# lincbrain/Fibers.jl

Hardware: AMD Instinct MI355X
Metric: Mvoxels/s fit (GQI ODF + peaks, 140^3 x 270-dir); Mpoints/s streamline in extra (higher is better)
Workload: dtype f32 (operands as 2 fp16 pieces = 23 bits on MFMA, 3 piece products, f32 accumulate); 1 GPU; gqi_rec + find_peaks + qa normalisation (gqi.jl:109-201), ONE 140x140x140 x 270-frame volume (18 x b=5 + 84 dirs x {1000,2000,3000}), sphere_642, all-ones mask; voxels=2744000, voxels_per_gpu=2744000, frames=270, odf_vertices=321, parallelism=single GPU

## Files before the change

### fibers.jl_amd/csrc/odf.hip

```cpp
#include <algorithm>
#include <cmath>
#include <type_traits>
#include <utility>

#include "common.h"

namespace {

typedef float f32x16 __attribute__((ext_vector_type(16)));

constexpr int KT = 16;
constexpr int WG_VOX = 128;

#include "odf_gemm_f32.inc"
#include "odf_fused_epilogue.inc"
#include "odf_gemm3.inc"
#include "odf_mask.inc"
#include "odf_peaks.inc"
#include "odf_post.inc"

}

struct fib_odf_plan {
    int device = 0;
    int nvol = 0, nvert = 0, nrows = 0, nrow0 = 0;
    int MB = 11, NX = 0, ntile_m = 1, Kpad = 0, maxdeg = 0;
    int scale_frame = -1;
    float scale_coef = 0.0f;
    bool has_ineff = false;
    int gM = 0, gK = 0, gRow0 = 0;
    std::vector<float> G;
    bool folded = false;
    int fold_span_max = 0, scale_frame_raw = -1;
    fib::DevBuf<int32_t> foldA, foldB;
    mutable fib::DevBuf<float> folded_dwi;
    std::vector<float> A;
    fib::DevBuf<float> At, verts;
    fib::DevBuf<uint16_t> At3;
    fib::DevBuf<float> Aextra;
    fib::DevBuf<float> Gdev;
    mutable fib::DevBuf<int32_t> inf_list;
    bool split_bf16 = false;
    bool h2 = false;
    float h2_sa = 1.0f;
    bool fused_shape = false;
    bool fused = false;
    bool dsi2_shape = false, dsi2 = false;
    int MBB = 0;
    fib::DevBuf<uint16_t> At3b;
    mutable fib::DevBuf<unsigned> pair_flags;
    fib::DevBuf<uint16_t> At3f;
    fib::DevBuf<float> Aextraf;
    mutable fib::DevBuf<float> mean_hi;
    mutable fib::DevBuf<int32_t> redo_list;
    fib::DevBuf<uint32_t> effbits;
    fib::DevBuf<int32_t> nbr, nbr64;
    int deg_pad = 6, rows_pad = 0;
    bool is_s642 = false;
    mutable fib::DevBuf<unsigned> maxenc;
    mutable fib::DevBuf<int32_t> live_vox, live_tiles, live_counts;
    mutable fib::DevBuf<unsigned long long> compact_state;
    mutable fib::DevBuf<unsigned long long> compact_sub;
    mutable fib::DevBuf<unsigned long long> compact_state2;
    mutable fib::DevBuf<unsigned> compact_mode;
    mutable fib::DevBuf<unsigned long long> compact_oct;
    mutable unsigned compact_epoch = 0;
    fib::DevBuf<unsigned> tickets;
    fib::DevBuf<unsigned> selctr;
    fib::DevBuf<unsigned long long> sellist;
    mutable fib::DevBuf<float> odfmax;
};

namespace {


int resolve_format(int format) {
    if (format != FIB_ODF_FORMAT_DEFAULT) return format;
    const char *e = fib::env("FIBERS_ODF_FORMAT");
    if (!e) {
        const char *g = fib::env("FIBERS_ODF_GEMM"), *x = fib::env("FIBERS_ODF_EXACT");
        if (g && (!strcmp(g, "f32") || !strcmp(g, "F32"))) return FIB_ODF_FORMAT_F32;
        if (x && x[0] != '\0' && x[0] != '0') return FIB_ODF_FORMAT_BF16X3;
    }
    if (e && (!strcmp(e, "f32") || !strcmp(e, "F32"))) return FIB_ODF_FORMAT_F32;
    if (e && (!strcmp(e, "bf16x3") || !strcmp(e, "BF16X3"))) return FIB_ODF_FORMAT_BF16X3;
    return FIB_ODF_FORMAT_FP16X2;
}

int finish_plan(fib_odf_plan *p, const float *verts, int nverts, const int32_t *faces, int nfaces,
                const std::vector<float> &frame_eff, int format = FIB_ODF_FORMAT_DEFAULT) {
    if (p->G.empty()) { p->G = p->A; p->gM = p->nrows; p->gK = p->nvol; p->gRow0 = p->nrow0; }
    const int M = p->gM, K = p->gK;
    format = resolve_format(format);
    p->split_bf16 = format != FIB_ODF_FORMAT_F32;
    int best_cost = INT32_MAX;
    const int nxs[] = {0, 1};
    for (int mb = p->split_bf16 ? 10 : 11; mb >= 5; mb--)
        for (int nx : nxs) {
            if (nx > 0 && mb > 10) continue;
            const int rows = mb * 32 + nx;
            const int nt = (M + rows - 1) / rows;
            const int cost = nt * (64 * mb + 4 * nx);
            if (cost < best_cost) { best_cost = cost; p->MB = mb; p->NX = nx; p->ntile_m = nt; }
        }
    p->Kpad = (K + KT - 1) / KT * KT;
    const int MW = gemm_row_stride(p->MB, p->NX), ROWS = p->MB * 32 + p->NX;
    std::vector<float> At((size_t)p->ntile_m * p->Kpad * MW, 0.0f);
    for (int k = 0; k < K; k++)
        for (int r = 0; r < M; r++) {
            const int tm = r / ROWS, rr = r % ROWS;
            At[((size_t)tm * p->Kpad + k) * MW + rr] = p->G[r + (size_t)M * k];
        }
    bool any_ineff = false;
    for (int k = 0; k < K; k++) if (frame_eff[k] == 0.0f) any_ineff = true;
    if (p->split_bf16 && (any_ineff || p->Kpad / KT < 2 || p->MB > 10 || (size_t)p->ntile_m * p->NX * p->Kpad > 2048)) p->split_bf16 = false;
    if (p->split_bf16) {
        p->h2 = format == FIB_ODF_FORMAT_FP16X2;
        float gmax = 0.0f;
// ... 254 lines not shown
            const float *cj = &p->A[(size_t)p->nrows * j], *ck = &p->A[(size_t)p->nrows * partner[j]];
            for (int r = 0; r < p->nrows && ok; r++) if (cj[r] != ck[r]) ok = false;
        }
        if (ok) {
            std::vector<int32_t> fa, fb;
            for (int j = 0; j < nvol; j++) if (j <= partner[j]) { fa.push_back(j); fb.push_back(partner[j] == j ? -1 : partner[j]); }
            const int nrep = (int)fa.size();
            p->folded = true; p->gK = nrep; p->gRow0 = nrep; p->gM = nrep + p->nvert;
            p->G.assign((size_t)p->gM * nrep, 0.0f);
            for (int c = 0; c < nrep; c++) {
                const float *col = &p->A[(size_t)p->nrows * fa[c]];
                for (int r = 0; r < nrep; r++) p->G[r + (size_t)p->gM * c] = col[fa[r]];
                for (int v = 0; v < p->nvert; v++) p->G[nrep + v + (size_t)p->gM * c] = col[nvol + v];
                if (fa[c] == p->scale_frame) p->scale_frame = -1000 - c;
            }
            if (p->scale_frame <= -1000) { p->scale_frame = -(p->scale_frame + 1000); p->scale_frame_raw = fa[p->scale_frame]; }
            for (int t0 = 0; t0 < nrep; t0 += KT)
                for (const std::vector<int32_t> *side : {&fa, &fb}) {
                    int lo = 1 << 30, hi = -1;
                    for (int j = t0; j < std::min(nrep, t0 + KT); j++) if ((*side)[j] >= 0) { lo = std::min(lo, (*side)[j]); hi = std::max(hi, (*side)[j]); }
                    if (hi >= 0) p->fold_span_max = std::max(p->fold_span_max, hi - lo + 1);
                }
            if ((rc = p->foldA.alloc(nrep)) != FIB_OK || (rc = p->foldB.alloc(nrep)) != FIB_OK) { delete p; return rc; }
            (void)hipMemcpy(p->foldA.p, fa.data(), nrep * sizeof(int32_t), hipMemcpyHostToDevice);
            (void)hipMemcpy(p->foldB.p, fb.data(), nrep * sizeof(int32_t), hipMemcpyHostToDevice);
            eff.assign((size_t)nrep, 1.0f);
        }
    }
    rc = finish_plan(p, verts, nverts, faces, nfaces, eff, format);
    if (rc != FIB_OK) { delete p; return rc; }
    *plan = p;
    return FIB_OK;
} FIB_API_CATCH

extern "C" void fib_odf_plan_destroy(fib_odf_plan *plan) try {
    if (!plan) return;
    fib::DeviceGuard guard;
    (void)hipSetDevice(plan->device);
    delete plan;
} FIB_API_CATCH_VOID

extern "C" int fib_odf_plan_matrix(const fib_odf_plan *plan, float *A, int *nrows, int *nvol, int *nvert) try {
    FIB_CHECK(plan != nullptr, FIB_ERR_INVALID, "plan is NULL");
    if (nrows) *nrows = plan->nrows;
    if (nvol) *nvol = plan->nvol;
    if (nvert) *nvert = plan->nvert;
    if (A) memcpy(A, plan->A.data(), plan->A.size() * sizeof(float));
    return FIB_OK;
} FIB_API_CATCH

namespace {

constexpr int FOLD_MB_MAX = 10;
template <int MB, int NX>
void launch_gemm(const GemmArgs &ga, unsigned grid, hipStream_t st) {
    if (ga.At3) {
        int ncu = 256, dev = 0;
        (void)hipGetDevice(&dev);
        (void)hipDeviceGetAttribute(&ncu, hipDeviceAttributeMultiprocessorCount, dev);
        GemmArgs g2 = ga;
        const int nw = 8;
        const int64_t items = fib::cdiv(ga.nvox, nw * 32) * ga.ntile_m;
        unsigned pg = (unsigned)std::min<int64_t>((int64_t)ncu * (8 / nw), items);
        pg = (pg + 7) / 8 * 8;
        auto go = [&](auto h2_) {
            constexpr bool H2 = decltype(h2_)::value;
            if (ga.fold) {
                if constexpr (MB <= FOLD_MB_MAX) hipLaunchKernelGGL((odf_gemm3_kernel<MB, NX, 8, true, false, H2>), dim3(pg), dim3(512), 0, st, g2);
                return;
            }
            if constexpr (MB == 10 && NX == 1) {
                if (ga.mean_hi) { hipLaunchKernelGGL((odf_gemm3_kernel<10, 1, 8, false, true, H2>), dim3(pg), dim3(512), 0, st, g2); return; }
            }
            hipLaunchKernelGGL((odf_gemm3_kernel<MB, NX, 8, false, false, H2>), dim3(pg), dim3(512), 0, st, g2);
        };
        if (ga.h2) go(std::true_type{}); else go(std::false_type{});
    }
    else hipLaunchKernelGGL((odf_gemm_kernel<MB, NX>), dim3(grid), dim3(256), 0, st, ga);
}

size_t peaks_smem(const fib_odf_plan *p) {
    return ((size_t)(p->rows_pad + 1) * PV + (size_t)PG * PV * PREC) * sizeof(float);
}

template <int DEG, bool EXACT>
int launch_peaks_t(const PeakArgs &pa, size_t smem, unsigned grid, hipStream_t st) {
    FIB_HIP(hipFuncSetAttribute(reinterpret_cast<const void *>(odf_peaks_kernel<DEG, EXACT>),
                                hipFuncAttributeMaxDynamicSharedMemorySize, (int)smem));
    hipLaunchKernelGGL((odf_peaks_kernel<DEG, EXACT>), dim3(grid), dim3(PW * 64), smem, st, pa);
    FIB_HIP(hipGetLastError());
    return FIB_OK;
}

template <int DEG, bool EXACT>
int launch_peaks64_t(const PeakArgs &pa, size_t smem, int64_t ntiles, unsigned grid, hipStream_t st) {
    FIB_HIP(hipFuncSetAttribute(reinterpret_cast<const void *>(odf_peaks64_kernel<DEG, EXACT>),
                                hipFuncAttributeMaxDynamicSharedMemorySize, (int)smem));
    hipLaunchKernelGGL((odf_peaks64_kernel<DEG, EXACT>), dim3(grid), dim3(P64_T), smem, st, pa, ntiles);
    FIB_HIP(hipGetLastError());
    return FIB_OK;
}

int launch_peaks(const fib_odf_plan *plan, const float *odf, int64_t nvox, int64_t stride, float *const peak[3], float *const qa[3],
                 int32_t *isort_top, int32_t *nvalid, bool reduce, hipStream_t st, bool small_tiles = false,
                 const int32_t *tiles = nullptr, const int32_t *ntl = nullptr) {
    PeakArgs pa{};
    pa.tiles = tiles; pa.ntl = ntl;
    pa.odf = odf; pa.nbr = plan->nbr.p; pa.nbr64 = plan->nbr64.p; pa.verts = plan->verts.p;
    for (int k = 0; k < 3; k++) { pa.peak[k] = peak ? peak[k] : nullptr; pa.qa[k] = qa ? qa[k] : nullptr; }
    pa.isort_top = isort_top; pa.nvalid = nvalid;
    pa.maxenc = reduce ? plan->maxenc.p : nullptr;
    pa.mean_hi = reduce ? plan->mean_hi.p : nullptr;
    pa.nvox = nvox; pa.stride = stride; pa.nvert = plan->nvert; pa.rows_pad = plan->rows_pad;
    pa.vec_ok = (stride % 4 == 0 && ((uintptr_t)odf & 15) == 0) ? 1 : 0;
    const size_t smem = peaks_smem(plan);
    FIB_CHECK(smem <= 160 * 1024, FIB_ERR_UNSUPPORTED, "ODF with %d vertices does not fit the peak finder's LDS tile", plan->nvert);
    const unsigned grid = (unsigned)fib::cdiv(nvox, PV);
    const bool exact = isort_top != nullptr;
    fib::ProfScope prof("odf_peaks", st);
    const size_t smem64 = ((size_t)(plan->nvert + 1) * 64 + (size_t)P64_W * 64 * PREC + (size_t)plan->nvert * (plan->deg_pad + 3)) * sizeof(float);
    if (!small_tiles && plan->nvert * 16 <= P64_NI * P64_T && smem64 <= 160 * 1024) {
        int ncu = 256;
        (void)hipDeviceGetAttribute(&ncu, hipDeviceAttributeMultiprocessorCount, plan->device);
        const int64_t ntiles = fib::cdiv(nvox, 64);
        const unsigned g64 = (unsigned)std::min<int64_t>(ntiles, ncu);
        if (plan->is_s642 && !exact) {
            const size_t smem642 = ((size_t)(FIB_S642_NVERT + 1) * 64 + (size_t)PQ_CAP * 64 * 2 + 128 + 2 * P64_W * 64 + 2 * 8 * 64 +
                                    (size_t)FIB_S642_NVERT * 3) * sizeof(float);
            FIB_HIP(hipFuncSetAttribute(reinterpret_cast<const void *>(odf_peaks642_kernel), hipFuncAttributeMaxDynamicSharedMemorySize, (int)smem642));
            hipLaunchKernelGGL(odf_peaks642_kernel, dim3(g64), dim3(P64_T), smem642, st, pa, ntiles);
            FIB_HIP(hipGetLastError());
            return FIB_OK;
        }
        switch (plan->deg_pad) {
            case 6:  return exact ? launch_peaks64_t<6, true>(pa, smem64, ntiles, g64, st) : launch_peaks64_t<6, false>(pa, smem64, ntiles, g64, st);
            case 8:  return exact ? launch_peaks64_t<8, true>(pa, smem64, ntiles, g64, st) : launch_peaks64_t<8, false>(pa, smem64, ntiles, g64, st);
            default: return exact ? launch_peaks64_t<16, true>(pa, smem64, ntiles, g64, st) : launch_peaks64_t<16, false>(pa, smem64, ntiles, g64, st);
        }
    }
    switch (plan->deg_pad) {
        case 6:  return exact ? launch_peaks_t<6, true>(pa, smem, grid, st) : launch_peaks_t<6, false>(pa, smem, grid, st);
        case 8:  return exact ? launch_peaks_t<8, true>(pa, smem, grid, st) : launch_peaks_t<8, false>(pa, smem, grid, st);
        default: return exact ? launch_peaks_t<16, true>(pa, smem, grid, st) : launch_peaks_t<16, false>(pa, smem, grid, st);
    }
}

}

namespace {
int launch_mask_compact(const fib_odf_plan *plan, const uint8_t *mask, int64_t nvox, unsigned *maxenc, const ZeroArgs *z, hipStream_t st) {
    int iters = (int)std::max<int64_t>(1, fib::cdiv(fib::cdiv(nvox, CB), 256));
    if (iters > CB_ITERS_MAX) iters = CB_ITERS_MAX;
    const int nchunks = (int)fib::cdiv(nvox, (int64_t)CB * iters);
    FIB_CHECK(nchunks <= 1024, FIB_ERR_UNSUPPORTED, "volume too large for the mask compaction");
    int rc;
    if ((rc = plan->live_vox.ensure((size_t)nvox)) != FIB_OK) return rc;
    if ((rc = plan->live_tiles.ensure((size_t)fib::cdiv(nvox, 64))) != FIB_OK) return rc;
    if (!plan->compact_state.p) {
        if ((rc = plan->compact_state.alloc(1024)) != FIB_OK) return rc;
        FIB_HIP(hipMemsetAsync(plan->compact_state.p, 0, 1024 * sizeof(unsigned long long), st));
    }
    if (!plan->compact_state2.p) {
        if ((rc = plan->compact_state2.alloc(1024)) != FIB_OK) return rc;
        FIB_HIP(hipMemsetAsync(plan->compact_state2.p, 0, 1024 * sizeof(unsigned long long), st));
        if ((rc = plan->compact_mode.alloc(2)) != FIB_OK) return rc;
        FIB_HIP(hipMemsetD32Async(reinterpret_cast<hipDeviceptr_t>(plan->compact_mode.p), 1, 2, st));
    }
    const size_t nsub = (size_t)fib::cdiv(nvox, CB);
    if (z && plan->compact_sub.n < nsub) {
        if ((rc = plan->compact_sub.alloc(nsub)) != FIB_OK) return rc;
        FIB_HIP(hipMemsetAsync(plan->compact_sub.p, 0, nsub * sizeof(unsigned long long), st));
    }
    if (++plan->compact_epoch == 0u) plan->compact_epoch = 1u;
    CompactArgs c{};
    c.mask = mask; c.nvox = nvox; c.vidx = plan->live_vox.p; c.tiles = plan->live_tiles.p; c.state = plan->compact_state.p;
    c.ticket = plan->tickets.p; c.totals = plan->live_counts.p; c.maxenc = maxenc; c.epoch = plan->compact_epoch; c.nchunks = nchunks; c.iters = iters;
    c.zero = z != nullptr;
    if (z) c.z = *z;
    c.clear = plan->pair_flags.p; c.nclear = plan->pair_flags.p ? 8 * 32 : 0;
    c.sub_state = plan->compact_sub.p;
    c.state2 = plan->compact_state2.p; c.mode = plan->compact_mode.p;
    const size_t noct = (size_t)fib::cdiv(nvox, 1024);
    if (z && noct * sizeof(unsigned) <= 48 * 1024) {
        if (plan->compact_oct.n < noct) {
            if ((rc = plan->compact_oct.alloc(noct)) != FIB_OK) return rc;
            FIB_HIP(hipMemsetAsync(plan->compact_oct.p, 0, noct * sizeof(unsigned long long), st));
        }
        c.oct_bits = plan->compact_oct.p; c.oct_words = (int)noct;
    }
    { const char *e = fib::ab_env("FIBERS_COMPACT_UNKNOWN"); c.dbg_unknown = e ? atoi(e) : 0; }
    { const char *e = fib::ab_env("FIBERS_ODF_LIST"); c.force = !e ? -1 : (e[0] == 'q' ? 0 : (e[0] == 'o' ? 1 : -1)); }
    fib::ProfScope prof("mask_compact", st);
    const int grid = nchunks + (z ? 256 : 0);
    hipLaunchKernelGGL(mask_compact_kernel, dim3(grid), dim3(1024), c.oct_words * sizeof(unsigned), st, c);
    FIB_HIP(hipGetLastError());
    return FIB_OK;
}
}

extern "C" int fibd_odf_rec(const fib_odf_plan *plan, const float *dwi, const uint8_t *mask, int64_t nvox,
                            float *pdf, float *odf, float *const peak[3], float *const qa[3],
                            float *odfmax_dev, int flags, void *stream) try {
    FIB_CHECK(plan && dwi && mask && odf && peak && qa, FIB_ERR_INVALID, "NULL argument");
    FIB_CHECK(nvox > 0, FIB_ERR_INVALID, "nvox must be positive");
    FIB_CHECK(nvox <= ((int64_t)1 << 27), FIB_ERR_UNSUPPORTED, "volumes of more than 2^27 voxels are not supported (32-bit lane offsets)");
    FIB_CHECK(plan->nrow0 == 0 || pdf != nullptr, FIB_ERR_INVALID, "DSI plans need a pdf output volume");
    for (int k = 0; k < 3; k++) FIB_CHECK(peak[k] && qa[k], FIB_ERR_INVALID, "NULL peak/qa output volume");
    fib::DeviceGuard guard;
    FIB_HIP(hipSetDevice(plan->device));
    hipStream_t st = (hipStream_t)stream;
    GemmArgs ga{};
    {
        ZeroArgs z{};
        z.out0 = pdf; z.out1 = odf; z.n0 = plan->nrow0; z.n1 = plan->nrows - plan->nrow0; z.nvox = nvox; z.stride = nvox;
        for (int k = 0; k < 3; k++) { z.peak[k] = peak[k]; z.qa[k] = qa[k]; }
        int rcc = launch_mask_compact(plan, mask, nvox, plan->maxenc.p, !(flags & FIB_ODF_PREZEROED) ? &z : nullptr, st);
        if (rcc != FIB_OK) return rcc;
    }
    ga.At = plan->At.p; ga.At3 = (plan->split_bf16 && nvox <= ((int64_t)1 << 26)) ? plan->At3.p : nullptr; ga.S = dwi;
    ga.Aextra = plan->Aextra.p; ga.h2 = plan->h2 ? 1 : 0; ga.h2_inv_sa = 1.0f / plan->h2_sa;
#ifdef FIB_CLOCK_STAMP
    { const char *pi = fib::ab_env("FIBERS_PHASE_ITEM"); ga.phase_item = pi ? atoi(pi) : 2; }
    { const char *pw = fib::ab_env("FIBERS_PHASE_WG"); ga.phase_wg = pw ? atoi(pw) : 8; }
#endif
    ga.vec_ok = (nvox % 4 == 0 && ((uintptr_t)odf & 15) == 0 && (pdf == nullptr || ((uintptr_t)pdf & 15) == 0)) ? 1 : 0; ga.vidx = plan->live_vox.p; ga.nlive = plan->live_counts.p; ga.mask = mask; ga.effbits = plan->effbits.p;
    ga.out0 = pdf; ga.out1 = odf; ga.nvox = nvox;
    if (ga.At3 && plan->Gdev.p) {
        int rci = plan->inf_list.ensure((size_t)nvox);
        if (rci != FIB_OK) return rci;
        ga.fix_count = plan->live_counts.p + 2; ga.fix_list = plan->inf_list.p; ga.fix_cap = (int)std::min<int64_t>(nvox, INT32_MAX);
    }
    const bool sep = (flags & FIB_ODF_SEPARATE_PEAKS) != 0;
    const bool fuse = plan->fused && ga.At3 != nullptr && ga.vec_ok && !sep;
    {
        int rcm = plan->mean_hi.ensure((size_t)nvox + 4);
        if (rcm != FIB_OK) return rcm;
    }
    auto setup_fused = [&]() -> int {
        int rcf = plan->redo_list.ensure((size_t)nvox);
        if (rcf != FIB_OK) return rcf;
        ga.At3 = plan->At3f.p; ga.Aextra = plan->Aextraf.p;
        for (int k = 0; k < 3; k++) { ga.peak[k] = peak[k]; ga.qa[k] = qa[k]; }
        ga.verts = plan->verts.p; ga.maxenc = plan->maxenc.p; ga.mean_hi = plan->mean_hi.p;
        ga.redo_count = plan->live_counts.p + 3; ga.redo_list = plan->redo_list.p; ga.redo_cap = (int)std::min<int64_t>(nvox, INT32_MAX);
        { const char *pa = fib::ab_env("FIBERS_ODF_ANTI"); ga.anti = pa ? atoi(pa) : 3; }
        return FIB_OK;
    };
    if (fuse) { int rcf = setup_fused(); if (rcf != FIB_OK) return rcf; }
    ga.K = plan->gK; ga.Kpad = plan->Kpad; ga.M = plan->gM; ga.nrow0 = plan->gRow0; ga.ntile_m = plan->ntile_m;
    const bool fold_ok = plan->folded && ga.At3 != nullptr && plan->Kpad <= FKMAX && plan->scale_frame_raw >= 0 &&
                         (int64_t)plan->fold_span_max * nvox * 4 < (int64_t)0xE0000000ll;
    const bool fuse_fold = fold_ok && plan->MB <= FOLD_MB_MAX;
    const bool dsi2 = plan->dsi2 && fold_ok && ga.vec_ok && !sep;
    if (dsi2) {
        int rcf = setup_fused();
        if (rcf != FIB_OK) return rcf;
        ga.At3b = plan->At3b.p;
        ga.ntile_m = 2;
    }
    if (fuse_fold || dsi2) {
        ga.fold = 1;
        ga.rowA = plan->foldA.p; ga.rowB = plan->foldB.p;
    } else if (plan->folded) {
        int rcf = plan->folded_dwi.ensure((size_t)plan->gK * nvox);
        if (rcf != FIB_OK) return rcf;
        fib::ProfScope prof("dsi_fold", st);
        if (nvox % 4 == 0 && ((uintptr_t)dwi & 15) == 0 && ((uintptr_t)mask & 3) == 0)
            hipLaunchKernelGGL(dsi_fold4_kernel, dim3((unsigned)fib::cdiv(nvox / 4, 256)), dim3(256), 0, st, dwi, mask, plan->foldA.p, plan->foldB.p,
                               plan->gK, nvox, plan->folded_dwi.p);
        else
            hipLaunchKernelGGL(dsi_fold_kernel, dim3((unsigned)fib::cdiv(nvox, 256)), dim3(256), 0, st, dwi, mask, plan->foldA.p, plan->foldB.p,
                               plan->gK, nvox, plan->folded_dwi.p);
        ga.S = plan->folded_dwi.p;
        ga.rowA = plan->foldA.p; ga.rowB = plan->foldB.p;
    }
    ga.scale_frame = plan->nrow0 > 0 ? ((fuse_fold || dsi2) ? plan->scale_frame_raw : plan->scale_frame) : -1;
    ga.scale_coef = plan->scale_coef;
    ga.stride = nvox;
    ga.has_ineff = plan->has_ineff ? 1 : 0;
    FIB_CHECK(fib::cdiv(nvox, WG_VOX) * plan->ntile_m < ((int64_t)1 << 31), FIB_ERR_UNSUPPORTED, "volume too large for one launch");

    auto run_gemm = [&](GemmArgs g, hipStream_t s) -> int {
        const unsigned grid = (unsigned)(fib::cdiv(g.nvox, WG_VOX) * plan->ntile_m);
        fib::ProfScope prof("odf_gemm", s);
        if (dsi2) {
            int ncu = 256;
            (void)hipDeviceGetAttribute(&ncu, hipDeviceAttributeMultiprocessorCount, plan->device);
            const int64_t items = fib::cdiv(g.nvox, 8 * 32) * 2;
            unsigned pg = (unsigned)std::min<int64_t>((int64_t)ncu, items);
            pg = (pg + 15) / 16 * 16;
            const int nslot = (int)pg / 8;
            const double ca = 68.0, cb = 19.0 + 4.5 * plan->MBB;
            int na = (int)(nslot * ca / (ca + cb) + 0.5);
            const char *ena = fib::ab_env("FIBERS_DSI_NA");
            if (ena) na = atoi(ena);
            g.dsi_na = std::max(1, std::min(nslot - 1, na));
            const char *epair = fib::ab_env("FIBERS_DSI_PAIR");
            if (plan->pair_flags.p && nslot <= 32 && !(epair && epair[0] == '0')) g.pair_flags = plan->pair_flags.p;
            switch (plan->MBB) {
                case 5: if (g.h2) hipLaunchKernelGGL((odf_dsi2_kernel<5, true>), dim3(pg), dim3(512), 0, s, g); else hipLaunchKernelGGL((odf_dsi2_kernel<5, false>), dim3(pg), dim3(512), 0, s, g); break;
                case 7: if (g.h2) hipLaunchKernelGGL((odf_dsi2_kernel<7, true>), dim3(pg), dim3(512), 0, s, g); else hipLaunchKernelGGL((odf_dsi2_kernel<7, false>), dim3(pg), dim3(512), 0, s, g); break;
                default: if (g.h2) hipLaunchKernelGGL((odf_dsi2_kernel<9, true>), dim3(pg), dim3(512), 0, s, g); else hipLaunchKernelGGL((odf_dsi2_kernel<9, false>), dim3(pg), dim3(512), 0, s, g); break;
            }
            FIB_HIP(hipGetLastError());
            return FIB_OK;
        }
#define FIB_GEMM_CASE(MBV, NXV) if (plan->MB == MBV && plan->NX == NXV) { launch_gemm<MBV, NXV>(g, grid, s); launched = true; }
        bool launched = false;
        FIB_GEMM_CASE(5, 0) FIB_GEMM_CASE(6, 0) FIB_GEMM_CASE(7, 0) FIB_GEMM_CASE(8, 0) FIB_GEMM_CASE(9, 0) FIB_GEMM_CASE(10, 0) FIB_GEMM_CASE(11, 0)
        FIB_GEMM_CASE(5, 1) FIB_GEMM_CASE(6, 1) FIB_GEMM_CASE(7, 1) FIB_GEMM_CASE(8, 1) FIB_GEMM_CASE(9, 1) FIB_GEMM_CASE(10, 1)
#undef FIB_GEMM_CASE
        if (!launched) return fib::fail(FIB_ERR_INVALID, "internal: no GEMM variant for MB=%d NX=%d", plan->MB, plan->NX);
        FIB_HIP(hipGetLastError());
        return FIB_OK;
    };

    int rc = run_gemm(ga, st);
    if (rc != FIB_OK) return rc;
    const bool fused_scan = fuse || dsi2;
    if (!fused_scan) {
        if (ga.fix_list) {
            InfFixArgs fx{plan->Gdev.p, dwi, odf, ga.fix_count, ga.fix_list, ga.fix_cap, plan->gM, plan->gK, nvox};
            hipLaunchKernelGGL(odf_inf_fix_kernel, dim3(64), dim3(256), 0, st, fx);
        }
        rc = launch_peaks(plan, odf, nvox, nvox, peak, qa, nullptr, nullptr, true, st, false, plan->live_tiles.p, plan->live_counts.p + 1);
        if (rc != FIB_OK) return rc;
    }
    float *om = odfmax_dev ? odfmax_dev : plan->odfmax.p;
    {
        fib::ProfScope prof("odf_post", st);
        PostArgs pa{};
        pa.redo = RedoArgs{odf, nvox, fused_scan ? ga.redo_count : nullptr, ga.redo_list, ga.redo_cap, plan->verts.p, {peak[0], peak[1], peak[2]}, {qa[0], qa[1], qa[2]}, plan->maxenc.p};
        pa.G = (fused_scan && ga.fix_list) ? plan->Gdev.p : nullptr; pa.S = dwi; pa.out = odf; pa.M = plan->gM; pa.K = plan->gK;
        pa.refine = RefineArgs{odf, nvox, nvox, plan->nvert, plan->live_vox.p, plan->live_counts.p, plan->mean_hi.p, plan->maxenc.p};
        pa.arrive = plan->tickets.p + 1; pa.odfmax = om; pa.raw = (flags & FIB_ODF_RAW_ODFMAX) ? 1 : 0;
        pa.selctr = plan->selctr.p; pa.sellist = plan->sellist.p; pa.selcap = POST_SELCAP; pa.epoch = plan->compact_epoch;
        if (flags & FIB_ODF_NORMALIZE) {
// ... 121 lines not shown
```

### fibers.jl_amd/csrc/odf_gemm3.inc

```

typedef __bf16 bf16x8_t __attribute__((ext_vector_type(8)));
typedef _Float16 f16x8_t __attribute__((ext_vector_type(8)));
typedef _Float16 f16x2_t __attribute__((ext_vector_type(2)));
typedef uint32_t u32x4_t __attribute__((ext_vector_type(4)));

__device__ __forceinline__ uint32_t cvt_pk_bf16(float lo, float hi) {
    uint32_t r;
    asm("v_cvt_pk_bf16_f32 %0, %1, %2" : "=v"(r) : "v"(lo), "v"(hi));
    return r;
}

constexpr int FKMAX = 512, FSMAX = FKMAX / KT;
template <int MB, int NX, int NW, bool FOLD, bool FUSE, bool H2, bool ONE = false>
constexpr int gemm3_lds_bytes() {
    constexpr bool SF = H2 && FOLD && ONE;
    return 2 * (H2 ? 2 : 3) * MB * 1024 + NW * (FUSE && !SF ? 4096 : 2048) + (NX > 0 ? (FUSE ? 2048 : 8192) : 0) +
           (FOLD ? 2 * FKMAX * 4 + 4 * FSMAX * 4 + (FUSE ? 0 : 2 * FKMAX * 4) : 0) + (FUSE ? NW * (SF ? FQ_LISTB : FQ_LIST) + FQ_TABB : 0) +
           (H2 && FUSE && !FOLD ? NW * (4096 + 512) : 0) +
           (SF ? NW * (8192 + 256) : 0);
}
template <int MB, int NX, int NW, bool FOLD = false, bool FUSE = false, bool ONE = false, bool H2 = false>
__device__ __forceinline__ void gemm3_body(const GemmArgs &a, char *lds) {
    static_assert(!FUSE || (MB == 10 && NX == 1), "the fused peak scan is generated for 10 blocks + 1 extra row");
    constexpr int NPIECE = (H2 ? 2 : 3) * MB;
// ... 424 lines not shown
                        kexp_fin = kexp;
                    }
                    if constexpr (SLDS) {
                        if (w1) { const bool in = t + 3 < ntiles; split(cur.tile_m, t + 1, (g + 1) & 1, in ? t + 3 : t + 3 - ntiles, in ? qoff : qoff_n, in || nxt.valid); }
                        else split(tm_n, 0, (g + 1) & 1, 2, qoff_n, nxt.valid);
                    } else {
                        split(tm_n, w1 ? t + 1 : 0);
                    }
                }
            }
            FIB_PHASE(g / ntiles, wave, 5);
            if constexpr (SLDS) { if (t > 0 || g == 0) __builtin_amdgcn_s_waitcnt(0x0F70 | NSREQ); }
            else
            __builtin_amdgcn_s_waitcnt(0x0F70);
            FIB_PHASE(g / ntiles, wave, 6);
            if constexpr (SLDS) __builtin_amdgcn_s_barrier();
            else
            __syncthreads();
            FIB_PHASE(g / ntiles, wave, 7);
        }
        if constexpr (SLDS) stage_A(nxt.valid ? nxt.tile_m : cur.tile_m, 1, (g & 1) ^ 1);
        {
            float vm = early ? vmax_fin : vmax;
            vm = max3_nan(vm, __shfl_xor(vm, 32), 0.0f);
            if (H2 && a.scale_frame < 0 && a.fix_list != nullptr && vm > 0.0f && vm < 1.17549435e-38f) vm = INFINITY;
            const float vn = vm < INFINITY ? 0.0f : __builtin_nanf("");
            const float asc = H2 ? __uint_as_float((uint32_t)(254 - (early ? kexp_fin : kexp)) << 23) * a.h2_inv_sa : 1.0f;
            if constexpr (FUSE) {
                float fscale = 1.0f;
                if (FOLD) { const float s0 = sraw < 0.0f ? 0.0f : sraw; fscale = vn != vn ? __builtin_nanf("") : 1.0f / (a.scale_coef * s0); }
                gemm3_epilogue_fused<NW, false, FOLD || H2, H2 && !FOLD, SLDS, SLDSF ? 1 : 2, SLDSF, SLDSF ? FQ_CAPB : FQ_CAP>(a, acc, early ? xfin[0] : xacc[0], vm, vn, inb, lv, vox, lane, lds + 2 * TILEB + wave * TRB,
                                                            lds + 2 * TILEB + NW * TRB + XTAB + FTAB + wave * QLIST, q_posoff, q_slotv, q_vl, en_run,
                                                            fscale * asc, fscale);
            }
            else {
                int le = lane;
                asm volatile("" : "+v"(le));
                if constexpr (SLDS) __builtin_amdgcn_s_waitcnt(0x0F70);
                if constexpr (FOLD)
                    gemm3_epilogue<MB, NX, false, 0, true, H2>(a, acc, xacc, vm, vn, inb, lv, vox, le, cur.tile_m, sraw, lds + 2 * TILEB + wave * TRB, f_row, f_row + FKMAX, asc);
                else
                    gemm3_epilogue<MB, NX, false, 0, false, H2>(a, acc, xacc, vm, vn, inb, lv, vox, le, cur.tile_m, sraw, lds + 2 * TILEB + wave * TRB, nullptr, nullptr, asc);
            }
        }
        FIB_PHASE(g / ntiles - 1, wave, 8);
        if (!nxt.valid) break;
        cur = nxt; inb = inb_n; vox = vox_n; s_off = s_off_n; qoff = qoff_n;
        nxt = work_at(g / ntiles + 1);
        if constexpr (SLDS) vraw_nxt = (int32_t)book[BOOKV + lane];
        else vraw_nxt = vidx_at(nxt);
        clear(early);
    }
    if constexpr (SLDS) __builtin_amdgcn_s_waitcnt(0x0F70);
    FIB_STAMP_END(ONE ? 8 : (FUSE ? 2 : (FOLD ? 3 : 1)), g / ntiles);
    if constexpr (FUSE) {
        for (int off = 32; off >= 1; off >>= 1) { const unsigned oth = (unsigned)__shfl_xor((int)en_run, off); en_run = oth > en_run ? oth : en_run; }
        if (lane == 0 && en_run) atomicMax(&a.maxenc[2], en_run);
    }
}

template <int MB, int NX, int NW, bool FOLD = false, bool FUSE = false, bool H2 = false>
__global__ __launch_bounds__(NW * 64, 2) void odf_gemm3_kernel(const GemmArgs a) {
    __shared__ __attribute__((aligned(16))) char lds[gemm3_lds_bytes<MB, NX, NW, FOLD, FUSE, H2>()];
    gemm3_body<MB, NX, NW, FOLD, FUSE, false, H2>(a, lds);
}

template <int MBB, bool H2>
__global__ __launch_bounds__(512, 2) void odf_dsi2_kernel(const GemmArgs a) {
    constexpr int LA_ = gemm3_lds_bytes<10, 1, 8, true, true, H2, true>(), LB_ = gemm3_lds_bytes<MBB, 0, 8, true, false, H2, true>();
    __shared__ __attribute__((aligned(16))) char lds[LA_ > LB_ ? LA_ : LB_];
    const int wslot = blockIdx.x >> 3, nslot = gridDim.x >> 3;
    GemmArgs b = a;
    const bool paired = a.pair_flags != nullptr && a.dsi_na <= 32;
    if (wslot < a.dsi_na) {
        b.one_slot = wslot; b.one_stride = a.dsi_na;
        b.pair_role = paired ? 1 : 0;
        gemm3_body<10, 1, 8, true, true, true, H2>(b, lds);
    } else {
        b.one_slot = wslot - a.dsi_na; b.one_stride = nslot - a.dsi_na;
        b.pair_role = paired ? 2 : 0;
        b.At3 = a.At3b;
        b.M = a.nrow0;
        gemm3_body<MBB, 0, 8, true, false, true, H2>(b, lds);
    }
}
```

### fibers.jl_amd/csrc/odf_gemm_f32.inc

```

struct GemmArgs {
    const float *At;
    const void *At3;
    const float *S;
    const int32_t *vidx;
    const int32_t *nlive;
    const uint8_t *mask;
    const uint32_t *effbits;
    float *out0;
    float *out1;
    int64_t nvox;
    int64_t stride;
    int K, Kpad, M, nrow0, ntile_m;
    int scale_frame;
    float scale_coef;
    int has_ineff;
    const float *Aextra;
    int vec_ok;
    const int32_t *rowA, *rowB;
    int32_t *fix_count, *fix_list;
    int fix_cap;
    int fold;
    float *peak[3], *qa[3];
    const float *verts;
    unsigned *maxenc;
    float *mean_hi;
    int32_t *redo_count, *redo_list;
    int redo_cap;
    int anti;
    const void *At3b;
    int one_slot, one_stride;
    int dsi_na;
    unsigned *pair_flags;
    int pair_role;
    int h2;
    float h2_inv_sa;
    int phase_item, phase_wg;
};

#ifdef FIB_CLOCK_STAMP
__device__ unsigned long long fib_clock_stamps[2048][4];
#define FIB_STAMP_BEGIN() unsigned long long fcs_c0_, fcs_r0_; asm volatile("s_memtime %0\n\ts_memrealtime %1\n\ts_waitcnt lgkmcnt(0)" : "=s"(fcs_c0_), "=s"(fcs_r0_) :: "memory")
#define FIB_STAMP_END(kid, items)                                                                                                   \
    do {                                                                                                                            \
        unsigned long long fcs_c1_, fcs_r1_;                                                                                        \
        asm volatile("s_memtime %0\n\ts_memrealtime %1\n\ts_waitcnt lgkmcnt(0)" : "=s"(fcs_c1_), "=s"(fcs_r1_) :: "memory");          \
        if (threadIdx.x == 0 && blockIdx.x < 2048) {                                                                                \
            fib_clock_stamps[blockIdx.x][0] = fcs_c1_ - fcs_c0_; fib_clock_stamps[blockIdx.x][1] = fcs_r1_ - fcs_r0_;               \
            fib_clock_stamps[blockIdx.x][2] = (kid); fib_clock_stamps[blockIdx.x][3] = (unsigned long long)(items);                 \
        }                                                                                                                           \
    } while (0)
__device__ unsigned long long fib_phase_stamps[2][256];
#ifdef FIB_PHASE_STAMP
#define FIB_PHASE_VARS() int fps_n_ = 0
#define FIB_PHASE(item_, wave_, id_)                                                                                                \
    do {                                                                                                                            \
        if ((int)blockIdx.x == a.phase_wg && (item_) == a.phase_item && ((wave_) & 3) == 0 && fps_n_ < 256) {                                     \
            unsigned long long t_;                                                                                                  \
            asm volatile("s_memtime %0\n\ts_waitcnt lgkmcnt(0)" : "=s"(t_) :: "memory");                                          \
            if ((threadIdx.x & 63) == 0) fib_phase_stamps[(wave_) >> 2][fps_n_] = (t_ << 8) | (unsigned)(id_);                      \
            fps_n_++;                                                                                                               \
        }                                                                                                                           \
    } while (0)
#else
#define FIB_PHASE_VARS() do { } while (0)
#define FIB_PHASE(item_, wave_, id_) do { } while (0)
#endif
#else
#define FIB_STAMP_BEGIN() do { } while (0)
#define FIB_STAMP_END(kid, items) do { } while (0)
#define FIB_PHASE_VARS() do { } while (0)
#define FIB_PHASE(item_, wave_, id_) do { } while (0)
#endif

template <int MB>
__device__ __forceinline__ void interleave_ds_mfma() {
#pragma unroll
    for (int i = 0; i < MB / 2; i++) {
        __builtin_amdgcn_sched_group_barrier(0x100, 1, 0);
        __builtin_amdgcn_sched_group_barrier(0x008, 2, 0);
    }
    if (MB & 1) {
        __builtin_amdgcn_sched_group_barrier(0x100, 1, 0);
        __builtin_amdgcn_sched_group_barrier(0x008, 1, 0);
    }
}

typedef float f32x2 __attribute__((ext_vector_type(2)));

__device__ __forceinline__ float clamp_sample(float x) {
// ... 385 lines not shown
```

### fibers.jl_amd/csrc/odf_mask.inc

```

constexpr int CB = 4096;
constexpr int CB_ITERS_MAX = 32;
__device__ __forceinline__ unsigned long long quad_expand(unsigned long long b) {
    unsigned long long q = (b | (b >> 1) | (b >> 2) | (b >> 3)) & 0x1111111111111111ull;
    return q | (q << 1) | (q << 2) | (q << 3);
}
__device__ __forceinline__ unsigned long long octet_expand(unsigned long long b) {
    return ((b & 0xffffffffull) ? 0xffffffffull : 0ull) | ((b >> 32) ? 0xffffffff00000000ull : 0ull);
}
struct ZeroArgs { float *out0, *out1, *peak[3], *qa[3]; int n0, n1; int64_t nvox, stride; };
struct CompactArgs {
    const uint8_t *mask; int64_t nvox;
    int32_t *vidx, *tiles;
    unsigned long long *state;
    unsigned *ticket;
    int32_t *totals;
    unsigned *maxenc;
    unsigned epoch;
    int nchunks, iters, zero;
    unsigned *clear; int nclear;
    unsigned long long *sub_state;
    unsigned long long *state2;
    unsigned *mode;
    int force;
    unsigned long long *oct_bits;
    int oct_words;
    int dbg_unknown;
    ZeroArgs z;
};
typedef __attribute__((address_space(1))) unsigned long long fib_gu64;
__global__ __launch_bounds__(1024) void mask_compact_kernel(const CompactArgs c) {
    __shared__ int cv[CB_ITERS_MAX][64], ct[CB_ITERS_MAX][64];
    __shared__ int s_chunk, s_base[2], s_agg[2], s_ndead[CB_ITERS_MAX], s_oct, s_alt[2], s_altsum[2];
    __shared__ unsigned s_gbits[CB_ITERS_MAX * 4];
    extern __shared__ unsigned s_octbits[];
    const int tid = threadIdx.x, lane = tid & 63, wave = tid >> 6;
    const bool compacts = (int)blockIdx.x < c.nchunks;
    if (compacts) {
        if (tid == 0) {
            s_chunk = (int)atomicAdd(c.ticket, 1u); s_base[0] = 0; s_base[1] = 0; s_alt[0] = 0; s_alt[1] = 0; s_altsum[0] = 0; s_altsum[1] = 0;
            s_oct = c.force >= 0 ? c.force : (c.mode ? (int)(c.mode[c.epoch & 1u] != 0u) : 0);
        }
        if (tid < CB_ITERS_MAX) s_ndead[tid] = 0;
        if (tid < CB_ITERS_MAX * 4) s_gbits[tid] = 0u;
        __syncthreads();
        const int t = s_chunk;
        const bool oct = s_oct != 0;
        const int64_t base = (int64_t)t * c.iters * CB;
        int nq = 0, no = 0;
        for (int it = 0; it < c.iters; it++) {
            int nd = 0;
#pragma unroll
            for (int i = 0; i < 4; i++) {
                const int64_t vx = base + (int64_t)it * CB + i * 1024 + tid;
                const unsigned long long inr = __ballot(vx < c.nvox);
                const unsigned long long b = __ballot(vx < c.nvox && c.mask[vx] != 0);
                const unsigned long long eq = quad_expand(b) & inr, eo = octet_expand(b) & inr;
                const unsigned long long e = oct ? eo : eq;
                nd += __popcll(inr & ~b);
                nq += __popcll(eq); no += __popcll(eo);
                if (lane == 0) { cv[it][i * 16 + wave] = __popcll(e); ct[it][i * 16 + wave] = b != 0ull; }
                if (lane == 0 && b) atomicOr(&s_gbits[it * 4 + i], (((b & 0xffffffffull) ? 1u : 0u) | ((b >> 32) ? 2u : 0u)) << (2 * wave));
            }
            if (c.zero && lane == 0 && nd) atomicAdd(&s_ndead[it], nd);
        }
        if (lane == 0 && c.state2) { atomicAdd(&s_alt[0], nq); atomicAdd(&s_alt[1], no); }
        __syncthreads();
        if (c.zero && oct && c.oct_bits && tid < c.iters * 4) {
            const int64_t gi = (base + (int64_t)(tid >> 2) * CB + (int64_t)(tid & 3) * 1024) >> 10;
            if (gi < c.oct_words)
                __hip_atomic_store((fib_gu64 *)(c.oct_bits + gi), ((unsigned long long)c.epoch << 32) | (unsigned long long)s_gbits[tid], __ATOMIC_RELAXED, __HIP_MEMORY_SCOPE_AGENT);
        }
        if (tid == 0 && c.state2)
            __hip_atomic_store((fib_gu64 *)(c.state2 + t), ((unsigned long long)(c.epoch & 0xfffffffu) << 36) | ((unsigned long long)s_alt[0] << 18) | (unsigned long long)s_alt[1],
                               __ATOMIC_RELAXED, __HIP_MEMORY_SCOPE_AGENT);
        if (c.zero && tid < c.iters && (int64_t)(t * c.iters + tid) * CB < c.nvox)
            __hip_atomic_store((fib_gu64 *)(c.sub_state + (size_t)t * c.iters + tid), ((unsigned long long)c.epoch << 32) | (unsigned)s_ndead[tid],
                               __ATOMIC_RELAXED, __HIP_MEMORY_SCOPE_AGENT);
        if (wave == 0) {
            int runv = 0, runt = 0;
            for (int it = 0; it < c.iters; it++) {
                const int v = cv[it][lane], tl = ct[it][lane];
                int sv = v, stl = tl;
#pragma unroll
                for (int off = 1; off < 64; off <<= 1) {
                    const int ov = __shfl_up(sv, off), ot = __shfl_up(stl, off);
                    if (lane >= off) { sv += ov; stl += ot; }
                }
                cv[it][lane] = runv + sv - v; ct[it][lane] = runt + stl - tl;
                runv += __shfl(sv, 63); runt += __shfl(stl, 63);
            }
            if (lane == 0) {
                s_agg[0] = runv; s_agg[1] = runt;
                __hip_atomic_store((fib_gu64 *)(c.state + t), ((unsigned long long)c.epoch << 32) | ((unsigned long long)runt << 18) | (unsigned long long)runv,
                                   __ATOMIC_RELAXED, __HIP_MEMORY_SCOPE_AGENT);
            }
        }
        {
            int pv = 0, pt = 0;
            if (tid < t) {
                unsigned long long g;
                for (;;) {
                    g = __hip_atomic_load((fib_gu64 *)(c.state + tid), __ATOMIC_RELAXED, __HIP_MEMORY_SCOPE_AGENT);
                    if ((unsigned)(g >> 32) == c.epoch) break;
                    __builtin_amdgcn_s_sleep(1);
                }
                pv = (int)(g & 0x3ffffull); pt = (int)((g >> 18) & 0x3fffull);
            }
#pragma unroll
            for (int off = 32; off >= 1; off >>= 1) { pv += __shfl_xor(pv, off); pt += __shfl_xor(pt, off); }
            if (lane == 0 && (pv | pt)) { atomicAdd(&s_base[0], pv); atomicAdd(&s_base[1], pt); }
        }
        if (t == c.nchunks - 1 && c.state2 && c.mode) {
            int aq = 0, ao = 0;
            if (tid <= t) {
                unsigned long long g;
                for (;;) {
                    g = __hip_atomic_load((fib_gu64 *)(c.state2 + tid), __ATOMIC_RELAXED, __HIP_MEMORY_SCOPE_AGENT);
                    if ((unsigned)(g >> 36) == (c.epoch & 0xfffffffu)) break;
                    __builtin_amdgcn_s_sleep(1);
                }
                aq = (int)((g >> 18) & 0x3ffffull); ao = (int)(g & 0x3ffffull);
            }
#pragma unroll
            for (int off = 32; off >= 1; off >>= 1) { aq += __shfl_xor(aq, off); ao += __shfl_xor(ao, off); }
            if (lane == 0 && (aq | ao)) { atomicAdd(&s_altsum[0], aq); atomicAdd(&s_altsum[1], ao); }
        }
        __syncthreads();
        if (t == c.nchunks - 1 && wave == 0) {
            if (lane == 0 && c.state2 && c.mode) c.mode[(c.epoch + 1u) & 1u] = (2ll * s_altsum[1] <= 3ll * s_altsum[0]) ? 1u : 0u;
            if (lane == 0) {
                c.totals[0] = s_base[0] + s_agg[0]; c.totals[1] = s_base[1] + s_agg[1]; c.totals[2] = 0; c.totals[3] = 0;
                if (c.maxenc) { c.maxenc[0] = 0u; c.maxenc[1] = 0u; c.maxenc[2] = 0u; c.maxenc[3] = 0u; }
                c.ticket[0] = 0u; c.ticket[1] = 0u;
            }
            for (int i = lane; i < c.nclear; i += 64) c.clear[i] = 0u;
        }
        for (int it = 0; it < c.iters; it++)
#pragma unroll
            for (int i = 0; i < 4; i++) {
                const int64_t vx = base + (int64_t)it * CB + i * 1024 + tid;
                const unsigned long long b = __ballot(vx < c.nvox && c.mask[vx] != 0);
                const unsigned long long e = (oct ? octet_expand(b) : quad_expand(b)) & __ballot(vx < c.nvox);
                const int pv = s_base[0] + cv[it][i * 16 + wave], pt = s_base[1] + ct[it][i * 16 + wave];
                if ((e >> lane) & 1ull) c.vidx[pv + __popcll(e & ((1ull << lane) - 1ull))] = (int32_t)vx;
                if (lane == 0 && b) c.tiles[pt] = (int32_t)(vx >> 6);
            }
        if (!c.zero) return;
    }
    const ZeroArgs &z = c.z;
    constexpr int ZS = 8, ZR = 16;
    __shared__ int s_nd[ZS], s_known, s_tot[2];
    const int nr = z.n0 + z.n1 + 12, ngrp = (nr + ZR - 1) / ZR;
    const int64_t nsub = (c.nvox + CB - 1) / CB, nspan = (nsub + ZS - 1) / ZS;
    const int hb = (int)blockIdx.x, nh = (int)gridDim.x;
    if (tid < 2) s_tot[tid] = 0;
    __syncthreads();
    {
        long long nd = 0;
        int unknown = 0;
        for (int64_t sidx = tid; sidx < nsub; sidx += 1024) {
            int got = -1;
            for (int spin = 0; spin < 600; spin++) {
                const unsigned long long w = __hip_atomic_load((fib_gu64 *)(c.sub_state + sidx), __ATOMIC_RELAXED, __HIP_MEMORY_SCOPE_AGENT);
                if ((unsigned)(w >> 32) == c.epoch) { got = (int)(unsigned)w; break; }
                __builtin_amdgcn_s_sleep(4);
            }
            if (got < 0) unknown = 1; else nd += got;
        }
        int q = (int)nd;
        for (int off = 32; off >= 1; off >>= 1) { q += __shfl_xor(q, off); unknown |= __shfl_xor(unknown, off); }
        if (lane == 0) { atomicAdd(&s_tot[0], q); if (unknown) atomicOr(&s_tot[1], 1); }
    }
    __syncthreads();
    const bool all_known = s_tot[1] == 0 && !(c.dbg_unknown > 0 && (int)blockIdx.x % c.dbg_unknown == 1);
    const int64_t total_dead = s_tot[0];
    if (all_known && total_dead == 0) return;
    const bool whole_ok = z.stride == c.nvox && (c.nvox & 3) == 0;
    const bool whole = all_known && total_dead * 4 > c.nvox && whole_ok;
    const bool both = !all_known && whole_ok;
    if (whole || both) {
        const bool octs = c.oct_bits != nullptr && c.oct_words > 0 && (c.force >= 0 ? c.force != 0 : (c.mode != nullptr && c.mode[c.epoch & 1u] != 0u));
        if (octs) {
            for (int gi = tid; gi < c.oct_words; gi += 1024) {
                unsigned bits = 0u;
// ... 179 lines not shown
```

Measured before the change: 1586 Mvoxels/s.

## Overlap zeroing of masked-out outputs with the fused GEMM in one launch

Instead of having the mask-compaction kernel zero the outputs of dead voxels, the compaction now publishes a per-quad liveness bitmap and a dead-quad count. A new fused GEMM launch splits its persistent workgroup slots between GEMM work and nontemporal zero-stores for dead quads, sized by a bytes-per-voxel cost model. The goal is to overlap the zero-fill traffic with GEMM compute. With the all-ones mask there are no dead voxels, so the kernel falls straight into the regular fused body, and the added cost is mostly the bitmap writes plus a different launch path.

```diff
diff --git a/fibers.jl_amd/csrc/odf.hip b/fibers.jl_amd/csrc/odf.hip
--- a/fibers.jl_amd/csrc/odf.hip
+++ b/fibers.jl_amd/csrc/odf.hip
@@ -64,6 +64,8 @@
     mutable fib::DevBuf<unsigned long long> compact_state2;
     mutable fib::DevBuf<unsigned> compact_mode;
     mutable fib::DevBuf<unsigned long long> compact_oct;
+    mutable fib::DevBuf<unsigned long long> clr_bits;
+    mutable fib::DevBuf<int32_t> clr_dead;
     mutable unsigned compact_epoch = 0;
     fib::DevBuf<unsigned> tickets;
     fib::DevBuf<unsigned> selctr;
@@ -424,17 +426,19 @@
 namespace {
 
 constexpr int FOLD_MB_MAX = 10;
+unsigned gemm3_grid(int64_t nvox, int ntile_m) {
+    int ncu = 256, dev = 0;
+    (void)hipGetDevice(&dev);
+    (void)hipDeviceGetAttribute(&ncu, hipDeviceAttributeMultiprocessorCount, dev);
+    const int64_t items = fib::cdiv(nvox, 8 * 32) * ntile_m;
+    const unsigned pg = (unsigned)std::min<int64_t>((int64_t)ncu, items);
+    return (pg + 7) / 8 * 8;
+}
 template <int MB, int NX>
 void launch_gemm(const GemmArgs &ga, unsigned grid, hipStream_t st) {
     if (ga.At3) {
-        int ncu = 256, dev = 0;
-        (void)hipGetDevice(&dev);
-        (void)hipDeviceGetAttribute(&ncu, hipDeviceAttributeMultiprocessorCount, dev);
         GemmArgs g2 = ga;
-        const int nw = 8;
-        const int64_t items = fib::cdiv(ga.nvox, nw * 32) * ga.ntile_m;
-        unsigned pg = (unsigned)std::min<int64_t>((int64_t)ncu * (8 / nw), items);
-        pg = (pg + 7) / 8 * 8;
+        const unsigned pg = gemm3_grid(ga.nvox, ga.ntile_m);
         auto go = [&](auto h2_) {
             constexpr bool H2 = decltype(h2_)::value;
             if (ga.fold) {
@@ -520,7 +524,7 @@
 }
 
 namespace {
-int launch_mask_compact(const fib_odf_plan *plan, const uint8_t *mask, int64_t nvox, unsigned *maxenc, const ZeroArgs *z, hipStream_t st) {
+int launch_mask_compact(const fib_odf_plan *plan, const uint8_t *mask, int64_t nvox, unsigned *maxenc, const ZeroArgs *z, hipStream_t st, bool publish = false) {
     int iters = (int)std::max<int64_t>(1, fib::cdiv(fib::cdiv(nvox, CB), 256));
     if (iters > CB_ITERS_MAX) iters = CB_ITERS_MAX;
     const int nchunks = (int)fib::cdiv(nvox, (int64_t)CB * iters);
@@ -560,6 +564,11 @@
         }
         c.oct_bits = plan->compact_oct.p; c.oct_words = (int)noct;
     }
+    if (publish && !z) {
+        if ((rc = plan->clr_bits.ensure((size_t)fib::cdiv(nvox, 256))) != FIB_OK) return rc;
+        if ((rc = plan->clr_dead.ensure(4)) != FIB_OK) return rc;
+        c.quad_bits = reinterpret_cast<unsigned short *>(plan->clr_bits.p); c.dead = plan->clr_dead.p;
+    }
     { const char *e = fib::ab_env("FIBERS_COMPACT_UNKNOWN"); c.dbg_unknown = e ? atoi(e) : 0; }
     { const char *e = fib::ab_env("FIBERS_ODF_LIST"); c.force = !e ? -1 : (e[0] == 'q' ? 0 : (e[0] == 'o' ? 1 : -1)); }
     fib::ProfScope prof("mask_compact", st);
@@ -582,28 +591,31 @@
     FIB_HIP(hipSetDevice(plan->device));
     hipStream_t st = (hipStream_t)stream;
     GemmArgs ga{};
+    ga.At = plan->At.p; ga.At3 = (plan->split_bf16 && nvox <= ((int64_t)1 << 26)) ? plan->At3.p : nullptr; ga.S = dwi;
+    ga.vec_ok = (nvox % 4 == 0 && ((uintptr_t)odf & 15) == 0 && (pdf == nullptr || ((uintptr_t)pdf & 15) == 0)) ? 1 : 0;
+    const bool sep = (flags & FIB_ODF_SEPARATE_PEAKS) != 0;
+    const bool fuse = plan->fused && ga.At3 != nullptr && ga.vec_ok && !sep;
+    bool clr = fuse && !(flags & FIB_ODF_PREZEROED) && gemm3_grid(nvox, plan->ntile_m) >= 16;
+    for (int k = 0; k < 3; k++) clr = clr && (((uintptr_t)peak[k] | (uintptr_t)qa[k]) & 15) == 0;
     {
         ZeroArgs z{};
         z.out0 = pdf; z.out1 = odf; z.n0 = plan->nrow0; z.n1 = plan->nrows - plan->nrow0; z.nvox = nvox; z.stride = nvox;
         for (int k = 0; k < 3; k++) { z.peak[k] = peak[k]; z.qa[k] = qa[k]; }
-        int rcc = launch_mask_compact(plan, mask, nvox, plan->maxenc.p, !(flags & FIB_ODF_PREZEROED) ? &z : nullptr, st);
+        int rcc = launch_mask_compact(plan, mask, nvox, plan->maxenc.p, (!(flags & FIB_ODF_PREZEROED) && !clr) ? &z : nullptr, st, clr);
         if (rcc != FIB_OK) return rcc;
     }
-    ga.At = plan->At.p; ga.At3 = (plan->split_bf16 && nvox <= ((int64_t)1 << 26)) ? plan->At3.p : nullptr; ga.S = dwi;
     ga.Aextra = plan->Aextra.p; ga.h2 = plan->h2 ? 1 : 0; ga.h2_inv_sa = 1.0f / plan->h2_sa;
 #ifdef FIB_CLOCK_STAMP
     { const char *pi = fib::ab_env("FIBERS_PHASE_ITEM"); ga.phase_item = pi ? atoi(pi) : 2; }
     { const char *pw = fib::ab_env("FIBERS_PHASE_WG"); ga.phase_wg = pw ? atoi(pw) : 8; }
 #endif
-    ga.vec_ok = (nvox % 4 == 0 && ((uintptr_t)odf & 15) == 0 && (pdf == nullptr || ((uintptr_t)pdf & 15) == 0)) ? 1 : 0; ga.vidx = plan->live_vox.p; ga.nlive = plan->live_counts.p; ga.mask = mask; ga.effbits = plan->effbits.p;
+    ga.vidx = plan->live_vox.p; ga.nlive = plan->live_counts.p; ga.mask = mask; ga.effbits = plan->effbits.p;
     ga.out0 = pdf; ga.out1 = odf; ga.nvox = nvox;
     if (ga.At3 && plan->Gdev.p) {
         int rci = plan->inf_list.ensure((size_t)nvox);
         if (rci != FIB_OK) return rci;
         ga.fix_count = plan->live_counts.p + 2; ga.fix_list = plan->inf_list.p; ga.fix_cap = (int)std::min<int64_t>(nvox, INT32_MAX);
     }
-    const bool sep = (flags & FIB_ODF_SEPARATE_PEAKS) != 0;
-    const bool fuse = plan->fused && ga.At3 != nullptr && ga.vec_ok && !sep;
     {
         int rcm = plan->mean_hi.ensure((size_t)nvox + 4);
         if (rcm != FIB_OK) return rcm;
@@ -655,6 +667,15 @@
     auto run_gemm = [&](GemmArgs g, hipStream_t s) -> int {
         const unsigned grid = (unsigned)(fib::cdiv(g.nvox, WG_VOX) * plan->ntile_m);
         fib::ProfScope prof("odf_gemm", s);
+        if (clr) {
+            g.clr_bits = plan->clr_bits.p; g.clr_dead = plan->clr_dead.p;
+            { const char *e = fib::ab_env("FIBERS_ODF_NCLR"); g.clr_force = e ? atoi(e) : -1; }
+            const unsigned pg = gemm3_grid(g.nvox, 1);
+            if (g.h2) hipLaunchKernelGGL((odf_gemm3_kernel_clr<true>), dim3(pg), dim3(512), 0, s, g);
+            else hipLaunchKernelGGL((odf_gemm3_kernel_clr<false>), dim3(pg), dim3(512), 0, s, g);
+            FIB_HIP(hipGetLastError());
+            return FIB_OK;
+        }
         if (dsi2) {
             int ncu = 256;
             (void)hipDeviceGetAttribute(&ncu, hipDeviceAttributeMultiprocessorCount, plan->device);
diff --git a/fibers.jl_amd/csrc/odf_gemm3.inc b/fibers.jl_amd/csrc/odf_gemm3.inc
--- a/fibers.jl_amd/csrc/odf_gemm3.inc
+++ b/fibers.jl_amd/csrc/odf_gemm3.inc
@@ -500,7 +500,7 @@
         clear(early);
     }
     if constexpr (SLDS) __builtin_amdgcn_s_waitcnt(0x0F70);
-    FIB_STAMP_END(ONE ? 8 : (FUSE ? 2 : (FOLD ? 3 : 1)), g / ntiles);
+    FIB_STAMP_END(ONE && FOLD ? 8 : (FUSE ? 2 : (FOLD ? 3 : 1)), g / ntiles);
     if constexpr (FUSE) {
         for (int off = 32; off >= 1; off >>= 1) { const unsigned oth = (unsigned)__shfl_xor((int)en_run, off); en_run = oth > en_run ? oth : en_run; }
         if (lane == 0 && en_run) atomicMax(&a.maxenc[2], en_run);
@@ -532,3 +532,58 @@
         gemm3_body<MBB, 0, 8, true, false, true, H2>(b, lds);
     }
 }
+
+constexpr int CLR_ROWS = FQ_NV + 9 + 3;
+constexpr int CLR_CHUNK = 37;
+static_assert(CLR_ROWS % CLR_CHUNK == 0, "clearing items are whole row chunks");
+constexpr float CLR_BYTES_PER_VOXEL = 7400.0f;
+__device__ __forceinline__ int clr_split(int nslot, int ndead, int nlive, int force) {
+    if (ndead <= 0) return 0;
+    const int cap = nslot >> 1;
+    int n;
+    if (force >= 0) n = force;
+    else if (nlive <= 0) n = cap;
+    else {
+        const float r = (float)ndead * (16.0f * CLR_ROWS / CLR_BYTES_PER_VOXEL) / (float)nlive;
+        n = (int)((float)nslot * r / (1.0f + r) + 0.5f);
+    }
+    return n < 1 ? 1 : (n > cap ? cap : n);
+}
+__device__ __forceinline__ void gemm3_clear_body(const GemmArgs &a, int cslot, int nclr) {
+    typedef float nt4_t __attribute__((ext_vector_type(4)));
+    const nt4_t zero4 = {0.0f, 0.0f, 0.0f, 0.0f};
+    const int lane = threadIdx.x & 63;
+    const int wave = __builtin_amdgcn_readfirstlane(threadIdx.x >> 6);
+    const int xcd = blockIdx.x & 7;
+    const int64_t nquad = a.nvox >> 2;
+    const int ngroup = (int)((nquad + 63) >> 6);
+    const int64_t nitem = (int64_t)ngroup * (CLR_ROWS / CLR_CHUNK);
+    const int nwave = nclr * 8 * 8;
+    for (int64_t item = (int64_t)((cslot * 8 + xcd) * 8 + wave); item < nitem; item += nwave) {
+        const int chunk = (int)(item / ngroup), group = (int)(item - (int64_t)chunk * ngroup);
+        const unsigned long long w = a.clr_bits[group];
+        const int64_t q = (int64_t)group * 64 + lane;
+        const bool dead = q < nquad && !((w >> lane) & 1ull);
+        if (!__any(dead)) continue;
+        for (int r = chunk * CLR_CHUNK; r < (chunk + 1) * CLR_CHUNK; r++) {
+            float *row;
+            if (r < FQ_NV) row = a.out1 + (int64_t)r * a.stride;
+            else if (r < FQ_NV + 9) { const int c = r - FQ_NV; row = a.peak[c / 3] + (int64_t)(c % 3) * a.stride; }
+            else row = a.qa[r - FQ_NV - 9];
+            if (dead) __builtin_nontemporal_store(zero4, reinterpret_cast<nt4_t *>(row) + q);
+        }
+    }
+}
+template <bool H2>
+__global__ __launch_bounds__(512, 2) void odf_gemm3_kernel_clr(const GemmArgs a) {
+    __shared__ __attribute__((aligned(16))) char lds[gemm3_lds_bytes<10, 1, 8, false, true, H2, true>()];
+    const int wslot = blockIdx.x >> 3, nslot = gridDim.x >> 3;
+    const int ndead = __builtin_amdgcn_readfirstlane(a.clr_dead[0]);
+    const int nlive = __builtin_amdgcn_readfirstlane(a.nlive[0]);
+    if (ndead <= 0) { gemm3_body<10, 1, 8, false, true, false, H2>(a, lds); return; }
+    const int nclr = clr_split(nslot, ndead, nlive, a.clr_force);
+    if (wslot >= nslot - nclr) { gemm3_clear_body(a, wslot - (nslot - nclr), nclr); return; }
+    GemmArgs b = a;
+    b.one_slot = wslot; b.one_stride = nslot - nclr; b.pair_role = 0;
+    gemm3_body<10, 1, 8, false, true, true, H2>(b, lds);
+}
diff --git a/fibers.jl_amd/csrc/odf_gemm_f32.inc b/fibers.jl_amd/csrc/odf_gemm_f32.inc
--- a/fibers.jl_amd/csrc/odf_gemm_f32.inc
+++ b/fibers.jl_amd/csrc/odf_gemm_f32.inc
@@ -36,6 +36,9 @@
     int h2;
     float h2_inv_sa;
     int phase_item, phase_wg;
+    const unsigned long long *clr_bits;
+    const int32_t *clr_dead;
+    int clr_force;
 };
 
 #ifdef FIB_CLOCK_STAMP
diff --git a/fibers.jl_amd/csrc/odf_mask.inc b/fibers.jl_amd/csrc/odf_mask.inc
--- a/fibers.jl_amd/csrc/odf_mask.inc
+++ b/fibers.jl_amd/csrc/odf_mask.inc
@@ -26,8 +26,17 @@
     unsigned long long *oct_bits;
     int oct_words;
     int dbg_unknown;
+    unsigned short *quad_bits;
+    int32_t *dead;
     ZeroArgs z;
 };
+__device__ __forceinline__ unsigned quad_bits16(unsigned long long e) {
+    unsigned long long x = e & 0x1111111111111111ull;
+    x = (x | (x >> 3)) & 0x0303030303030303ull;
+    x = (x | (x >> 6)) & 0x000f000f000f000full;
+    x = (x | (x >> 12)) & 0x000000ff000000ffull;
+    return (unsigned)((x | (x >> 24)) & 0xffffull);
+}
 typedef __attribute__((address_space(1))) unsigned long long fib_gu64;
 __global__ __launch_bounds__(1024) void mask_compact_kernel(const CompactArgs c) {
     __shared__ int cv[CB_ITERS_MAX][64], ct[CB_ITERS_MAX][64];
@@ -61,6 +70,7 @@
                 nq += __popcll(eq); no += __popcll(eo);
                 if (lane == 0) { cv[it][i * 16 + wave] = __popcll(e); ct[it][i * 16 + wave] = b != 0ull; }
                 if (lane == 0 && b) atomicOr(&s_gbits[it * 4 + i], (((b & 0xffffffffull) ? 1u : 0u) | ((b >> 32) ? 2u : 0u)) << (2 * wave));
+                if (c.quad_bits && lane == 0 && inr) c.quad_bits[vx >> 6] = (unsigned short)quad_bits16(e);
             }
             if (c.zero && lane == 0 && nd) atomicAdd(&s_ndead[it], nd);
         }
@@ -131,6 +141,7 @@
             if (lane == 0 && c.state2 && c.mode) c.mode[(c.epoch + 1u) & 1u] = (2ll * s_altsum[1] <= 3ll * s_altsum[0]) ? 1u : 0u;
             if (lane == 0) {
                 c.totals[0] = s_base[0] + s_agg[0]; c.totals[1] = s_base[1] + s_agg[1]; c.totals[2] = 0; c.totals[3] = 0;
+                if (c.dead) c.dead[0] = (int32_t)((c.nvox - (int64_t)(s_base[0] + s_agg[0])) >> 2);
                 if (c.maxenc) { c.maxenc[0] = 0u; c.maxenc[1] = 0u; c.maxenc[2] = 0u; c.maxenc[3] = 0u; }
                 c.ticket[0] = 0u; c.ticket[1] = 0u;
             }
```

After: 1547 Mvoxels/s. -2.5%, worse.
